# HeyWeCome/WhisprRec

Measured on AMD Instinct MI355X. Metric: BPR training triplets/sec, higher is better.
Workload: dtype f32; 1 GPU; BPRMF emb_size=64, synthetic 1000000 users x 1000000 items (uniform ids), batch 65536, SGD l2=0, plan build in timed region; batch=65536, emb_size=64, optimizer=SGD, plan_chunk_batches=64, tables=single GPU, step_stream=whisprrec_amd.hip_ops.PipelinedSgd, plan=group plan (no per-batch sort: flags + lists of the shared rows, wr_group.hip), chained_step_launch=True, plan_build=on a side stream, beside the steps of the chunk before

## Files before the change

include/whisprrec_hip.h:

```cpp
#ifndef WHISPRREC_HIP_H
#define WHISPRREC_HIP_H

#include <stdint.h>

#ifdef __cplusplus
extern "C" {
#endif

#define WR_ABI_VERSION 1

#define WR_OK 0
#define WR_E_NULL (-1)
#define WR_E_SHAPE (-2)
#define WR_E_WORKSPACE (-3)
#define WR_E_ALIGN (-4)
#define WR_E_RANGE (-5)

int32_t wr_abi_version(void);
const char *wr_last_error(void);
int32_t wr_device_info(int32_t *n_cu, int32_t *wave_size, char *arch, int32_t arch_len);

int64_t wr_bpr_fwd_workspace_bytes(int64_t B);
int32_t wr_bpr_fwd(const float *user_tab, int64_t n_users, const float *item_tab, int64_t n_items, int32_t D,
                   const int64_t *u, const int64_t *p, const int64_t *n, int64_t B, float *pos_score, float *neg_score,
// ... 143 lines not shown

int64_t wr_group_plan_words(int64_t n_triplets, int64_t batch_size, int64_t n_users, int64_t n_items);
int32_t wr_group_plan_layout(int64_t n_triplets, int64_t batch_size, int64_t n_users, int64_t n_items, int64_t *out);
int32_t wr_narrow_ids_i64(const int64_t *u, const int64_t *p, const int64_t *n, int32_t *u32, int32_t *p32, int32_t *n32,
                          int64_t count, void *stream);
int32_t wr_group_plan_build(const int32_t *u, const int32_t *p, const int32_t *n, int64_t n_triplets, int64_t batch_size,
                            int64_t n_users, int64_t n_items, int32_t *plan, int64_t plan_words, void *stream);
int64_t wr_bprmf_group_workspace_bytes(int64_t batch_size, int32_t D);
int64_t wr_bprmf_group_sync_words(int64_t n_batches);
int32_t wr_bprmf_group_supported(const float *user_tab, const float *item_tab, int32_t D);
int32_t wr_bprmf_run_sgd_group(float *user_tab, int64_t n_users, float *item_tab, int64_t n_items, int32_t D,
                               const int32_t *u, const int32_t *p, const int32_t *n, int64_t n_triplets, int64_t batch_size,
                               const int32_t *plan, int64_t plan_words, int64_t first_batch, int64_t n_batches, float lr,
                               float *loss_out, void *const *events, void *workspace, int64_t workspace_bytes, int32_t *sync,
                               int64_t sync_words, void *stream);

int32_t wr_bprmf_plan_overlap_marks(const int32_t *tu, const int32_t *tp, const int32_t *tn, int64_t n_triplets,
                                    int64_t batch_size, int64_t n_items, const int32_t *prev_bitmap, int32_t *bitmap,
                                    int32_t *tdef, int32_t *def_q, int64_t def_cap, int32_t *def_count, void *stream);

int32_t wr_bprmf_plan_overlap_deferred(const int32_t *tu, const int32_t *tp, const int32_t *tn, int64_t n_triplets,
                                       int64_t batch_size, int64_t n_items, const int32_t *prev_bitmap, const int32_t *bitmap,
                                       int32_t *tdef, int32_t *def_q, int64_t def_cap, int32_t *def_count, void *stream);

int32_t wr_bprmf_grads(const float *user_tab, int64_t n_users, const float *item_tab, int64_t n_items, int32_t D,
                       const int32_t *tu, const int32_t *tp, const int32_t *tn, const int32_t *oc_item,
                       const int32_t *oc_src, int64_t B, float *grad_u, float *grad_i, int32_t *stamp_u,
                       int32_t *stamp_i, int32_t step_id, float *loss_out, const wr_hot_runs *hot, void *workspace,
                       int64_t workspace_bytes, void *stream);

// ... 208 lines not shown
```

whisprrec_amd/abi.py:

```python
import ctypes
import os

_HERE = os.path.dirname(os.path.abspath(__file__))
LIB_PATH = os.path.join(_HERE, "libwhisprrec_hip.so")

c_i32, c_i64, c_f32, c_vp = ctypes.c_int32, ctypes.c_int64, ctypes.c_float, ctypes.c_void_p

SIGNATURES = {
    "wr_abi_version": (c_i32, []),
    "wr_last_error": (ctypes.c_char_p, []),
    "wr_device_info": (c_i32, [c_vp, c_vp, c_vp, c_i32]),
    "wr_bpr_fwd_workspace_bytes": (c_i64, [c_i64]),
    "wr_bpr_fwd": (c_i32, [c_vp, c_i64, c_vp, c_i64, c_i32, c_vp, c_vp, c_vp, c_i64, c_vp, c_vp, c_vp, c_vp, c_vp, c_i64,
                           c_vp]),
    "wr_bprmf_plan_workspace_bytes": (c_i64, [c_i64, c_i64, c_i64, c_i64]),
    "wr_bprmf_plan_build_i64": (c_i32, [c_vp, c_vp, c_vp, c_i64, c_i64, c_i64, c_i64, c_vp, c_vp, c_vp, c_vp, c_vp, c_vp,
                                        c_vp, c_vp, c_i64, c_vp]),
    "wr_bprmf_plan_build_i32": (c_i32, [c_vp, c_vp, c_vp, c_i64, c_i64, c_i64, c_i64, c_vp, c_vp, c_vp, c_vp, c_vp, c_vp,
                                        c_vp, c_vp, c_i64, c_vp]),
    "wr_bprmf_plan_small_max_batch": (c_i64, []),
    "wr_bprmf_plan_build_small_i64": (c_i32, [c_vp, c_vp, c_vp, c_i64, c_i64, c_i64, c_i64, c_vp, c_vp, c_vp, c_vp, c_vp, c_vp,
                                              c_vp, c_vp]),
    "wr_bprmf_plan_build_small_i32": (c_i32, [c_vp, c_vp, c_vp, c_i64, c_i64, c_i64, c_i64, c_vp, c_vp, c_vp, c_vp, c_vp, c_vp,
                                              c_vp, c_vp]),
# ... 48 lines not shown
                                 c_i64, c_f32, c_i32, c_vp, c_vp, c_vp, c_vp, c_i64, c_vp]),
    "wr_shard_route": (c_i32, [c_vp, c_vp, c_vp, c_i64, c_i64, c_i32, c_i32, c_i64, c_i64, c_i64, c_i64, c_i64, c_vp, c_vp, c_vp,
                               c_vp, c_vp, c_vp, c_vp]),
    "wr_shard_pack": (c_i32, [c_vp, c_vp, c_i64, c_i32, c_i64, c_i64, c_vp, c_i64, c_vp, c_vp, c_vp]),
    "wr_bprmf_shard_step_group": (c_i32, [c_vp, c_i64, c_vp, c_i64, c_i64, c_i32, c_vp, c_vp, c_vp, c_i64, c_i64, c_vp, c_i64,
                                          c_i64, c_i64, c_f32, c_vp, c_vp, c_vp, c_i64, c_vp, c_i64, c_vp]),
    "wr_group_plan_words": (c_i64, [c_i64, c_i64, c_i64, c_i64]),
    "wr_group_plan_layout": (c_i32, [c_i64, c_i64, c_i64, c_i64, c_vp]),
    "wr_narrow_ids_i64": (c_i32, [c_vp, c_vp, c_vp, c_vp, c_vp, c_vp, c_i64, c_vp]),
    "wr_group_plan_build": (c_i32, [c_vp, c_vp, c_vp, c_i64, c_i64, c_i64, c_i64, c_vp, c_i64, c_vp]),
    "wr_bprmf_group_workspace_bytes": (c_i64, [c_i64, c_i32]),
    "wr_bprmf_group_sync_words": (c_i64, [c_i64]),
    "wr_bprmf_group_supported": (c_i32, [c_vp, c_vp, c_i32]),
    "wr_bprmf_run_sgd_group": (c_i32, [c_vp, c_i64, c_vp, c_i64, c_i32, c_vp, c_vp, c_vp, c_i64, c_i64, c_vp, c_i64, c_i64,
                                       c_i64, c_f32, c_vp, c_vp, c_vp, c_i64, c_vp, c_i64, c_vp]),
    "wr_bprmf_plan_overlap_deferred": (c_i32, [c_vp, c_vp, c_vp, c_i64, c_i64, c_i64, c_vp, c_vp, c_vp, c_vp, c_i64, c_vp,
                                               c_vp]),
    "wr_bprmf_plan_fast_marks_supported": (c_i32, [c_i64, c_i64, c_i64, c_i64]),
    "wr_bprmf_plan_build_fast_marks_i64": (c_i32, [c_vp, c_vp, c_vp, c_i64, c_i64, c_i64, c_i64, c_vp, c_vp, c_vp, c_vp, c_vp,
                                                   c_vp, c_vp, c_vp, c_i64, c_vp, c_vp]),
    "wr_bprmf_plan_build_fast_marks_i32": (c_i32, [c_vp, c_vp, c_vp, c_i64, c_i64, c_i64, c_i64, c_vp, c_vp, c_vp, c_vp, c_vp,
                                                   c_vp, c_vp, c_vp, c_i64, c_vp, c_vp]),
    "wr_bprmf_plan_overlap_marks": (c_i32, [c_vp, c_vp, c_vp, c_i64, c_i64, c_i64, c_vp, c_vp, c_vp, c_vp, c_i64, c_vp,
                                            c_vp]),
    "wr_bprmf_grads": (c_i32, [c_vp, c_i64, c_vp, c_i64, c_i32, c_vp, c_vp, c_vp, c_vp, c_vp, c_i64, c_vp, c_vp, c_vp,
                               c_vp, c_i32, c_vp, c_vp, c_vp, c_i64, c_vp]),
    "wr_sgd_decay_untouched": (c_i32, [c_vp, c_i64, c_i32, c_vp, c_i32, c_f32, c_f32, c_vp]),
    "wr_sgd_dense": (c_i32, [c_vp, c_i64, c_i32, c_vp, c_vp, c_i32, c_f32, c_f32, c_vp]),
    "wr_adam_dense": (c_i32, [c_vp, c_vp, c_vp, c_i64, c_i32, c_vp, c_vp, c_i32, c_i64, c_f32, c_f32, c_f32, c_f32,
                              c_f32, c_vp]),
# ... 77 lines not shown



class HotRuns(ctypes.Structure):
    _fields_ = [("piece_q", c_vp), ("piece_len", c_vp), ("run_q", c_vp), ("run_first", c_vp), ("run_np", c_vp),
                ("u_piece_q", c_vp), ("u_piece_len", c_vp), ("u_run_q", c_vp), ("u_run_first", c_vp), ("u_run_np", c_vp),
                ("counts_host", c_vp), ("cap_pieces", c_i64), ("cap_runs", c_i64), ("cap_u_pieces", c_i64),
                ("cap_u_runs", c_i64)]


class DenseGroup(ctypes.Structure):
    _fields_ = [("A_T", c_vp), ("cols", c_vp), ("rows", c_vp), ("partials", c_vp), ("K_pad", c_i64), ("k_per_split", c_i64),
                ("n_tiles", c_i64)]


class BucketSide(ctypes.Structure):
    _fields_ = [("n_buckets", c_i32), ("row_bucket", c_vp), ("bucket_start", c_vp), ("bucket_rows", c_vp), ("bucket_sub", c_vp)]


_lib = None


class WhisprRecHipError(RuntimeError):
    pass


def lib():
    global _lib
    if _lib is None:
        if not os.path.exists(LIB_PATH):
# ... 29 lines not shown
```

whisprrec_amd/csrc/wr_group.hip:

```cpp
#include "wr_common.h"
#include <hip/hip_ext.h>

#include <algorithm>

namespace wr {

constexpr int kGpThreads = 1024;
constexpr unsigned kGpRangeBits = 18;
constexpr int kGpWords = 1 << (kGpRangeBits - 5);
constexpr int kGpCap = 8192;
constexpr int kGpBins = 4096;
constexpr int kGpMaxBin = 256;
constexpr int kGpMaxRanges = 8;
constexpr int64_t kGpMaxBatch = 1 << 17;
constexpr int kGpLongRun = 64;
constexpr int kGpMetaWords = 16;
#ifndef WR_GP_DBG
#define WR_GP_DBG 0
#endif

struct GroupLayout {
    int64_t nb, B, fw;
    int R_u, R_i, cap_u, cap_i;
    unsigned mask_u, mask_i, hbits_u, hbits_i;
// ... 669 lines not shown
#define WR_GS_NIT 1024
#endif

struct GroupRun {
    TablePair tabs;
    const int32_t *u, *p, *n, *plan;
    int64_t n_triplets, batch_size, plan_words, workspace_bytes, sync_words;
    BatchRange range;
    float lr, *loss_out;
    void *const *events;
    void *workspace;
    uint32_t *sync;
    int n_cu;
    float *grad_slots;
    int64_t n_local_items, global_batch;
    hipStream_t stream;
};

template <int T, int NV, bool FULL>
static int32_t launch_group_steps(const GroupRun &g, const GroupLayout &L, const GpDev &G) {
    const int32_t D = g.tabs.D;
    const int64_t n_batches = g.range.n_batches, global_batch = g.global_batch;
    uint32_t *const sync = g.sync;
    const int64_t B = L.B;
    const int64_t ws_one = gs_ws_one(B, D), zb = align_up(B * (int64_t)D * 4, 256);
    char *ws = reinterpret_cast<char *>(g.workspace);
    float *Zs[2] = {reinterpret_cast<float *>(ws), reinterpret_cast<float *>(ws + ws_one)};
    float *ZUs[2] = {reinterpret_cast<float *>(ws + zb), reinterpret_cast<float *>(ws + ws_one + zb)};
    float *Ps[2] = {reinterpret_cast<float *>(ws + 2 * zb), reinterpret_cast<float *>(ws + ws_one + 2 * zb)};
    constexpr int TEAMS = kBlock / T;
    WR_HIP(hipMemsetAsync(sync, 0, (size_t)(n_batches * kGsStepWords) * 4, g.stream));
    uint32_t *timeout = sync + (g.sync_words - 4);
    int nDS = WR_GS_NDS;
    while (nDS > g.n_cu / 4 && nDS > 1) nDS >>= 1;
    auto batch_of = [&](int64_t b) {
        const int64_t off = b * B;
        const int Bk = (int)batch_len(g.n_triplets, B, b);
        return GsBatch{g.u + off, g.p + off, g.n + off, reinterpret_cast<const uint4 *>(G.flags + b * L.fw * 4),
                       G.ul_row + b * L.R_u * (int64_t)L.cap_u, G.ul_src + b * L.R_u * (int64_t)L.cap_u, G.ucnt + b * L.R_u,
                       G.il_row + b * L.R_i * (int64_t)L.cap_i, G.il_src + b * L.R_i * (int64_t)L.cap_i, G.icnt + b * L.R_i,
                       Bk, L.R_u, L.R_i, L.cap_u, L.cap_i};
    };
    auto ev = [&](int64_t k, int j) { return g.events ? reinterpret_cast<hipEvent_t>(g.events[2 * k + j]) : (hipEvent_t) nullptr; };
    int n_partials_prev = 0;
    for (int64_t k = 0; k <= n_batches; ++k) {
        GsArgs a{};
        a.U = g.tabs.U;
        a.I = g.tabs.I;
        a.D = D;
        a.lr = g.lr;
        a.done = sync + (k < n_batches ? k : 0) * kGsStepWords;
        a.timeout = timeout;
        a.Gs = g.grad_slots;
        a.nL = (int)g.n_local_items;
        const bool have_cur = k < n_batches, have_prev = k > 0;
        if (have_cur) {
            a.cur = batch_of(g.range.first_batch + k);
            a.Z = Zs[k & 1];
            a.ZU = ZUs[k & 1];
            a.partials = Ps[k & 1];
            a.denom = global_batch > 0 ? (float)global_batch : (float)a.cur.B;
            a.nA = (int)((a.cur.B + TEAMS - 1) / TEAMS);
            a.nDS = have_prev ? nDS : 0;
            a.chained = have_prev ? 1 : 0;
        }
        if (have_prev) {
            a.prev = batch_of(g.range.first_batch + k - 1);
            a.Zp = Zs[(k - 1) & 1];
            a.ZUp = ZUs[(k - 1) & 1];
            a.partials_prev = Ps[(k - 1) & 1];
            a.n_partials_prev = n_partials_prev;
            a.denom_prev = global_batch > 0 ? (float)global_batch : (float)a.prev.B;
            a.loss_prev = at_or_null(g.loss_out, k - 1);
            a.nIT = (int)std::min<int64_t>(WR_GS_NIT, (2 * B + kGsTile - 1) / kGsTile + L.R_i);
            a.nUT = (int)std::min<int64_t>(WR_GS_NUT, (B + kGsTile - 1) / kGsTile + L.R_u);
        }
        a.tiles_at = (int)((int64_t)a.nA * WR_GS_TILES_AT / 16);
        a.side_at = std::max(a.tiles_at, (int)((int64_t)a.nA * WR_GS_SIDE_AT / 16));
        const dim3 grid((unsigned)(a.nA + a.nIT + a.nUT + a.nDS));
        hipEvent_t e0 = have_cur ? ev(k, 0) : nullptr, e1 = have_cur ? ev(k, 1) : nullptr;
        if (e0 != nullptr || e1 != nullptr)
            hipExtLaunchKernelGGL((bprmf_group_step<T, NV, FULL>), grid, dim3(kBlock), 0, g.stream, e0, e1, 0, a);
        else
            hipLaunchKernelGGL((bprmf_group_step<T, NV, FULL>), grid, dim3(kBlock), 0, g.stream, a);
        WR_LAUNCH_CHECK("bprmf_group_step");
        n_partials_prev = a.nA + a.nDS;
    }
    return WR_OK;
}

static int32_t check_group_plan(const char *entry, const GroupRun &g, GroupLayout &L) {
    int32_t rc;
    if ((rc = check_whole_lines(entry, whole_lines(g.tabs.U, g.tabs.I, g.tabs.D), g.tabs.D)) != WR_OK) return rc;
    WR_REQUIRE(group_layout(g.n_triplets, g.batch_size, g.tabs.n_users, g.tabs.n_items, L), WR_E_RANGE,
               "group plan not applicable to n=%lld, batch=%lld", (long long)g.n_triplets, (long long)g.batch_size);
    WR_REQUIRE(g.plan_words >= L.total, WR_E_WORKSPACE, "group plan: %lld words < %lld", (long long)g.plan_words, (long long)L.total);
    return WR_OK;
}

static int32_t run_group(const char *entry, GroupRun &g, const GroupLayout &L, int64_t sync_batches) {
    int32_t rc;
    if ((rc = check_workspace(entry, g.workspace, g.workspace_bytes, 2 * gs_ws_one(g.batch_size, g.tabs.D))) != WR_OK) return rc;
    if ((rc = check_sync_words(entry, g.sync, g.sync_words, sync_batches * kGsStepWords + 4)) != WR_OK) return rc;
    if (g.range.n_batches == 0) return WR_OK;
    if (g.n_cu == 0 && (rc = device_cu_count(&g.n_cu)) != WR_OK) return rc;
    const GpDev G = group_dev(const_cast<int32_t *>(g.plan), L);
#define WR_CALL_GS(T_, NV_, FULL_) return launch_group_steps<T_, NV_, FULL_>(g, L, G)
    WR_DISPATCH_D(g.tabs.D, WR_CALL_GS);
#undef WR_CALL_GS
    return WR_OK;
}

}

using namespace wr;

extern "C" {

int64_t wr_group_plan_words(int64_t n_triplets, int64_t batch_size, int64_t n_users, int64_t n_items) {
    GroupLayout L;
    if (!group_layout(n_triplets, batch_size, n_users, n_items, L)) return 0;
// ... 66 lines not shown
    g.plan = plan; g.plan_words = plan_words;
    g.range = BatchRange{first_batch, n_batches};
    g.lr = lr; g.loss_out = loss_out; g.events = events;
    g.workspace = workspace; g.workspace_bytes = workspace_bytes;
    g.sync = reinterpret_cast<uint32_t *>(sync); g.sync_words = sync_words;
    g.stream = reinterpret_cast<hipStream_t>(stream);
    int32_t rc;
    GroupLayout L;
    if ((rc = check_tables(g.tabs)) != WR_OK) return rc;
    WR_REQUIRE(u && p && n && plan && sync, WR_E_NULL, "index arrays / plan / sync words must not be NULL");
    if ((rc = check_group_plan("wr_bprmf_run_sgd_group", g, L)) != WR_OK) return rc;
    WR_REQUIRE(first_batch >= 0 && n_batches >= 0 && first_batch + n_batches <= L.nb, WR_E_SHAPE,
               "batches [%lld,%lld) exceed the plan's %lld", (long long)first_batch, (long long)(first_batch + n_batches),
               (long long)L.nb);
    return run_group("wr_bprmf_run_sgd_group", g, L, n_batches + 1);
}

int32_t wr_bprmf_shard_step_group(float *user_shard, int64_t n_user_rows, float *item_ext, int64_t n_ext_rows,
                                  int64_t n_local_items, int32_t D, const int32_t *vu, const int32_t *vp, const int32_t *vn,
                                  int64_t n_triplets, int64_t batch_size, const int32_t *plan, int64_t plan_words, int64_t batch,
                                  int64_t global_batch, float lr, float *grad_slots, float *loss_partial, void *workspace,
                                  int64_t workspace_bytes, int32_t *sync, int64_t sync_words, void *stream) {
    GroupRun g{};
    g.tabs = TablePair{user_shard, item_ext, n_user_rows, n_ext_rows, D};
    g.u = vu; g.p = vp; g.n = vn; g.n_triplets = n_triplets; g.batch_size = batch_size;
    g.plan = plan; g.plan_words = plan_words;
    g.range = BatchRange{batch, 1};
    g.lr = lr; g.loss_out = loss_partial;
    g.workspace = workspace; g.workspace_bytes = workspace_bytes;
    g.sync = reinterpret_cast<uint32_t *>(sync); g.sync_words = sync_words;
// ... 19 lines not shown
```

whisprrec_amd/hip_ops.py:

```python
import ctypes

import torch

from . import abi


def _stream():
    return torch.cuda.current_stream().cuda_stream


def _p(t):
    return None if t is None else t.data_ptr()


def _addr(struct):
    return ctypes.addressof(struct) if struct is not None else None


def _event_handles(events, per_step, count, allow_none):
    if events is None:
        return None
    if len(events) != per_step * count:
        raise ValueError("%s must hold %d events per step" % ("phase_events" if per_step == 4 else "events", per_step))
    handles = []
# ... 522 lines not shown

    def __init__(self, u, p, n, batch_size, n_users, n_items, arena=None, defer=False):
        u, p, n = (_req(t, torch.int32, nm, 1) for t, nm in ((u, "u"), (p, "p"), (n, "n")))
        N = u.numel()
        if not (p.numel() == N and n.numel() == N) or N == 0:
            raise ValueError("u/p/n must have the same non-zero length")
        L = abi.lib()
        self.u, self.p, self.n = u, p, n
        self.n_triplets, self.batch_size = N, int(batch_size)
        self.n_users, self.n_items = int(n_users), int(n_items)
        self.n_batches = (N + self.batch_size - 1) // self.batch_size
        self.words = int(L.wr_group_plan_words(N, self.batch_size, self.n_users, self.n_items))
        if self.words <= 0:
            raise abi.WhisprRecHipError("group plan: shape not supported (batch size %d)" % self.batch_size)
        self.arena = arena
        self._stream = torch.cuda.current_stream(u.device)
        if arena is not None:
            if arena.buf.numel() < self.words or arena.batch_size != self.batch_size or \
                    (arena.n_users, arena.n_items) != (self.n_users, self.n_items):
                raise ValueError("plan does not fit its arena")
            if arena.free is not None:
                self._stream.wait_event(arena.free)
                arena.free = None
            self.buf = arena.buf
            self._pinned = arena.meta_host
        else:
            self.buf = torch.empty(self.words, dtype=torch.int32, device=u.device)
            self._pinned = None
        abi.check(L.wr_group_plan_build(_p(u), _p(p), _p(n), N, self.batch_size, self.n_users, self.n_items, _p(self.buf),
                                        self.buf.numel(), _stream()), "wr_group_plan_build")
# ... 193 lines not shown
        return bufs[-1]

    def run_sgd_group(self, gplan, first, count, lr, losses=None, events=None):
        L = abi.lib()
        nbytes = abi.check_size(L.wr_bprmf_group_workspace_bytes(gplan.batch_size, self.D), "wr_bprmf_group_workspace_bytes")
        ws = workspace(self.dev, "group_step").get(nbytes)
        losses = self._loss_buf(losses, count)
        ev = _event_handles(events, 2, count, False)
        sync = self._group_sync(count)
        abi.check(L.wr_bprmf_run_sgd_group(*self._table_head(), _p(gplan.u), _p(gplan.p), _p(gplan.n), gplan.n_triplets,
                                           gplan.batch_size, _p(gplan.buf), gplan.buf.numel(), first, count, lr, _p(losses),
                                           _addr(ev), _p(ws), ws.numel(), _p(sync), sync.numel(), _stream()),
                  "wr_bprmf_run_sgd_group")
        self.step_id += count
        return losses

    def grads(self, plan, k, grad_u, grad_i, loss_out=None, stamps=True):
        L = abi.lib()
        ws = self._ws(plan.batch_size)
        su, si = self._stamps() if stamps else (None, None)
        loss_out = self._loss_buf(loss_out)
        self.step_id += 1
        hot = plan.hot_struct(k)
        abi.check(L.wr_bprmf_grads(*self._table_head(), *self._plan_ptrs(plan, k), _p(grad_u), _p(grad_i), _p(su), _p(si),
                                   self.step_id, _p(loss_out), _addr(hot), _p(ws), ws.numel(), _stream()), "wr_bprmf_grads")
        return loss_out, self.step_id


PAIR_SET_MIN_PAIRS = 1 << 20

# ... 293 lines not shown
    if adjacent:
        return torch.as_strided(a, (end - a.storage_offset(),), (1,), a.storage_offset())
    return torch.cat(ts)


class PipelinedSgd:

    PREFETCH_AFTER_TRIPLETS = 0
    PLAN_TRIPLETS = 1 << 22
    GROUP_MIN_ROWS_PER_TRIPLET = 12
    GROUP_MIN_BATCH = 4096

    CHAIN_MIN_BATCH = 8192
    CHAIN_MIN_ITEMS_PER_TRIPLET = 6

    def __init__(self, chunk=64, min_triplets=None, chain=True, inline_plan=False, group=True):
        import sys
        self.ops = sys.modules[__name__]
        self.chunk = int(chunk)
        self.chain = bool(chain)
        self.group = bool(group)
        self.inline_plan = inline_plan
        self.stats = {"plain_calls": 0, "chain_calls": 0, "group_calls": 0, "group_fallbacks": 0}
        self._garenas = {}
        if min_triplets is not None:
            self.PLAN_TRIPLETS = int(min_triplets)
        self.plan_stream = None
        self._arenas = {}

    def chunk_batches(self, batch_size):
        return max(self.chunk, self.PLAN_TRIPLETS // max(int(batch_size), 1))

    def _arena_pair(self, device, B, nb_total, overlap_items):
        cap = min(self.chunk_batches(B), max(int(nb_total), 1)) * B
        key = (str(device), B, int(overlap_items))
        pair = self._arenas.get(key)
        if pair is None or pair[0].max_triplets < cap:
            pair = [self.ops.PlanArena(device, cap, B, overlap_items=overlap_items) for _ in range(2)]
            self._arenas[key] = pair
        return pair

    def _garena_pair(self, device, B, nb_total, n_users, n_items):
        cap = min(self.chunk_batches(B), max(int(nb_total), 1)) * B
        key = (str(device), B, int(n_users), int(n_items))
        pair = self._garenas.get(key)
        if pair is None or pair[0].max_triplets < cap:
            pair = [self.ops.GroupArena(device, cap, B, n_users, n_items) for _ in range(2)]
            self._garenas[key] = pair
        return pair

    def plan(self, U, segments, batch, first_chunk=None, lr=None, prep=None, runner=None):
        if self.plan_stream is None:
            self.plan_stream = side_stream(U.device)
        B = int(batch)
        segs, first = [], 0
        for k, (rows, u, p, n) in enumerate(segments):
            nb = (u.numel() + B - 1) // B
            if u.numel() % B != 0 and any(s[1].numel() for s in segments[k + 1:]):
                raise ValueError("only the last segment may end with a short batch")
            segs.append({"tabs": self.ops.BprmfTables(U, rows) if nb else None, "nb": nb, "first": first})
            first += nb
        live = [s for s in segments if s[1].numel()]
# ... 3 lines not shown
        use_chain = self.chain and (runner is None or getattr(runner, "wants_chain_marks", False)) and \
            B >= self.CHAIN_MIN_BATCH and first >= 2 and \
            min([s[0].shape[0] for s in live] or [0]) >= self.CHAIN_MIN_ITEMS_PER_TRIPLET * B and \
            all(sg["tabs"].chain_supported() for sg in segs if sg["tabs"] is not None)
        min_rows = min([U.shape[0]] + [s[0].shape[0] for s in live])
        use_group = self.group and runner is None and len(live) == 1 and first >= 2 and \
            self.GROUP_MIN_BATCH <= B <= 131072 and u_all.dtype in (torch.int32, torch.int64) and \
            min_rows >= self.GROUP_MIN_ROWS_PER_TRIPLET * B and \
            all(sg["tabs"].group_supported() for sg in segs if sg["tabs"] is not None)
        garenas = self._garena_pair(U.device, B, first, U.shape[0], n_items) if use_group else None
        arenas = None if use_group else self._arena_pair(U.device, B, first, n_items if use_chain else 0)
        for a in (arenas or []) + (garenas or []):
            a.release_after(main)
        h = {"segs": segs, "B": B, "u": u_all, "p": p_all, "n": n_all, "nb": first, "n_users": U.shape[0], "n_items": n_items,
             "at": 0, "tag": 0, "next": None, "cur": None, "map": None, "arenas": arenas, "pos": 0,
             "group": use_group, "garenas": garenas, "device": U.device,
             "ids32": [torch.empty(u_all.numel(), dtype=torch.int32, device=U.device) for _ in range(3)]
                      if use_group and u_all.dtype == torch.int64 else None,
             "chain": use_chain, "prep": prep, "runner": runner, "inline": bool(self.inline_plan),
             "lead": [int(c) for c in (first_chunk if isinstance(first_chunk, (list, tuple)) else [first_chunk or 0]) if c]}
        self.plan_stream.wait_stream(main)
        self._prefetch(h)
        return h

    def _build_stream(self, h):
        return torch.cuda.current_stream(h["u"].device) if h["inline"] else self.plan_stream

    def _prefetch(self, h):
        if h["at"] >= h["nb"]:
            h["next"] = None
            return
# ... 1 lines not shown
        c = min(self.chunk_batches(B), h["nb"] - first)
        if h["lead"]:
            c = min(c, h["lead"].pop(0))
        h["at"] += c
        lo, hi = first * B, min(h["u"].numel(), (first + c) * B)
        with torch.cuda.stream(self._build_stream(h)):
            bmap = h["map"] if h["map"] else None
            if h["prep"] is not None:
                h["prep"].fill(lo, hi)
            if h["group"]:
                cols = (h["u"], h["p"], h["n"])
                if h["ids32"] is not None:
                    abi.check(abi.lib().wr_narrow_ids_i64(*[_p(c[lo:hi]) for c in cols], *[_p(c[lo:hi]) for c in h["ids32"]],
                                                          hi - lo, _stream()), "wr_narrow_ids_i64")
                    cols = h["ids32"]
                plan = self.ops.GroupPlan(cols[0][lo:hi], cols[1][lo:hi], cols[2][lo:hi], B, h["n_users"], h["n_items"],
                                          arena=h["garenas"][h["tag"]], defer=True)
                h["tag"] ^= 1
                h["next"] = (first, plan)
                return
            if h["arenas"] is None:
                h["arenas"] = self._arena_pair(h["device"], B, h["nb"], h["n_items"] if h["chain"] else 0)
            plan = self.ops.BatchPlan(h["u"][lo:hi], h["p"][lo:hi], h["n"][lo:hi], B, h["n_users"], h["n_items"],
                                      validate=False, ws_tag="rot%d" % h["tag"], bucket_map=bmap, arena=h["arenas"][h["tag"]],
                                      defer=True, overlap=h["chain"])
        h["tag"] ^= 1
        h["next"] = (first, plan)

    STICKY_MSG = "a wait inside a step launch expired (hand-off between the workgroups of one launch): the tables are not " \
                 "valid — do not save or evaluate them; restart the run"

    def _queue_sticky(self, h, tabs, main):
        words = tabs.sticky_words()
        if not words:
            return
        pin = h.get("sticky_pin")
        if pin is None or pin.numel() < 2 * len(words):
            pin = h["sticky_pin"] = torch.zeros(2 * max(len(words), 4), dtype=torch.int32, pin_memory=True)
        half = pin.numel() // 2
        off = half * (h.get("sticky_tag", 0) & 1)
        h["sticky_tag"] = h.get("sticky_tag", 0) + 1
        for j, wd in enumerate(words):
            pin[off + j:off + j + 1].copy_(wd, non_blocking=True)
        ev = torch.cuda.Event()
        ev.record(main)
        self._check_sticky(h)
        h["sticky_pending"] = (ev, pin[off:off + len(words)])

    def _check_sticky(self, h):
        pend = h.pop("sticky_pending", None)
        if pend is not None:
            pend[0].synchronize()
            if bool(pend[1].numpy().any()):
                raise abi.WhisprRecHipError(self.STICKY_MSG)

    def _take_next(self, h, pos, main):
        self._check_sticky(h)
        if h["next"] is None:
            self._prefetch(h)
        cur = h["next"]
        assert cur is not None and cur[0] == pos, "steps must be run in order"
        plan = cur[1]
        plan.validate()
        if isinstance(plan, GroupPlan):
            if plan.overflow or plan.long_run:
                h["group"] = False
                self.stats["group_fallbacks"] += 1
                if h["next"] is not None and h["next"][0] != cur[0]:
                    raise AssertionError("plan pipeline out of step")
                if plan.overflow:
                    first, B = cur[0], h["B"]
                    lo, hi = first * B, first * B + plan.n_triplets
                    plan.arena.release_after(main)
                    if h["arenas"] is None:
                        h["arenas"] = self._arena_pair(h["device"], B, h["nb"], h["n_items"] if h["chain"] else 0)
                    with torch.cuda.stream(self._build_stream(h)):
                        plan = self.ops.BatchPlan(h["u"][lo:hi], h["p"][lo:hi], h["n"][lo:hi], B, h["n_users"], h["n_items"],
                                                  validate=False, ws_tag="rot%d" % h["tag"], arena=h["arenas"][h["tag"]],
                                                  defer=True, overlap=h["chain"])
                    h["tag"] ^= 1
                    plan.validate()
                    cur = (first, plan)
            main.wait_event(plan.ready)
            h["cur"], h["next"] = cur, None
            return cur
        main.wait_event(plan.ready)
        if plan.fast_overflowed:
# ... 17 lines not shown
        while pos < end:
            cur = h["cur"]
            if cur is None or pos >= cur[0] + cur[1].n_batches:
                cur = self._take_next(h, pos, main)
            base, plan = cur
            c = min(end, base + plan.n_batches) - pos
            if h["inline"] and h["next"] is None and h["at"] < h["nb"]:
                mid = base + plan.n_batches // 2
                if pos >= mid:
                    self._prefetch(h)
                else:
                    c = min(c, mid - pos)
            elif self.PREFETCH_AFTER_TRIPLETS > 0 and h["next"] is None and h["at"] < h["nb"] and \
                    c > (self.PREFETCH_AFTER_TRIPLETS + h["B"] - 1) // h["B"]:
                c = (self.PREFETCH_AFTER_TRIPLETS + h["B"] - 1) // h["B"]
            if isinstance(plan, GroupPlan):
                sg["tabs"].run_sgd_group(plan, pos - base, c, lr, losses=losses[loss_off:loss_off + c])
                self.stats["group_calls"] += 1
            elif h["runner"] is not None:
                h["runner"](plan, pos - base, c, losses[loss_off:loss_off + c])
                self.stats["plain_calls"] += 1
            elif h["chain"] and plan.overlap is not None and c >= 2:
                sg["tabs"].run_sgd_chain(plan, pos - base, c, lr, losses=losses[loss_off:loss_off + c])
                self.stats["chain_calls"] += 1
            else:
                sg["tabs"].run_sgd(plan, pos - base, c, lr, losses=losses[loss_off:loss_off + c])
                self.stats["plain_calls"] += 1
            pos += c
            loss_off += c
            if pos >= base + plan.n_batches:
                plan.arena.release_after(main)
                self._queue_sticky(h, sg["tabs"], main)
            if h["next"] is None and not h["inline"]:
                self._prefetch(h)
        h["pos"] = pos

    def run(self, handle, seg, lr, losses):
        sg = handle["segs"][seg]
        if sg["nb"] == 0:
            return
        self._run_span(handle, sg, sg["first"], sg["first"] + sg["nb"], lr, losses, 0)
        if seg == len(handle["segs"]) - 1:
            self._check_sticky(handle)

    def run_steps(self, handle, count, lr, losses):
        assert len(handle["segs"]) == 1, "run_steps: single-segment handles"
        sg = handle["segs"][0]
        pos = handle["pos"]
        if pos + count > sg["nb"]:
            raise ValueError("run_steps: %d steps asked, %d left" % (count, sg["nb"] - pos))
        self._run_span(handle, sg, pos, pos + count, lr, losses, 0)


class LazyOptimizerState:

    FOLD_MAX_GAP = 40

    MAX_LAG = 64
    LAG_MIN_GAP = 64

    def __init__(self, tabs, name, lr, l2, betas=(0.9, 0.999), eps=1e-8, fold=None, max_lag=None):
        self.chain, self.chain_calls = True, 0
        if name not in ("SGD", "Adam"):
            raise ValueError(name)
        self.tabs, self.name, self.lr, self.l2, self.betas, self.eps = tabs, name, float(lr), float(l2), betas, float(eps)
        self.fold = fold if fold is None else bool(fold)
# ... 477 lines not shown
```

Baseline: 2.587 billion triplets/s.

## Carry the last batch's deferred update across group-plan chunk boundaries

The chained group step normally finishes the previous batch's scatter inside the next batch's kernel, but each call drained the pipeline with a tail launch at the chunk end. A carry struct now holds the last batch's plan pointers, buffer half and partial counts, so the next chunk's first step applies it chained instead of in a standalone drain. Each plan is built with one lead-in batch so row-sharing lists cover the boundary, and a third arena keeps the carried plan alive. A flush entry point drains the carry on fallback, lr or table change, and at run end. It also batches the sticky-word device-to-host copies into one copy, at the cost of more bookkeeping and a larger plan per chunk.

After: 2.633 billion triplets/s (median of 6 runs). 1.02x the previous value.

```diff
diff --git a/include/whisprrec_hip.h b/include/whisprrec_hip.h
--- a/include/whisprrec_hip.h
+++ b/include/whisprrec_hip.h
@@ -181,6 +181,31 @@
                                const int32_t *plan, int64_t plan_words, int64_t first_batch, int64_t n_batches, float lr,
                                float *loss_out, void *const *events, void *workspace, int64_t workspace_bytes, int32_t *sync,
                                int64_t sync_words, void *stream);
+
+typedef struct wr_group_carry {
+    const int32_t *u, *p, *n;
+    const void *flags;
+    const int32_t *ul_row, *ul_src, *ul_cnt, *il_row, *il_src, *il_cnt;
+    int32_t B, R_u, R_i, cap_u, cap_i;
+    int32_t valid;
+    int32_t half;
+    int32_t n_partials;
+    float denom, lr;
+    float *loss;
+    const void *user_tab, *item_tab, *workspace;
+    int32_t D;
+    int32_t reserved;
+    int64_t batch_size;
+} wr_group_carry;
+int32_t wr_bprmf_run_sgd_group_carry(float *user_tab, int64_t n_users, float *item_tab, int64_t n_items, int32_t D,
+                                     const int32_t *u, const int32_t *p, const int32_t *n, int64_t n_triplets,
+                                     int64_t batch_size, const int32_t *plan, int64_t plan_words, int64_t first_batch,
+                                     int64_t n_batches, float lr, float *loss_out, void *const *events, void *workspace,
+                                     int64_t workspace_bytes, int32_t *sync, int64_t sync_words, wr_group_carry *carry,
+                                     int32_t carry_in, int32_t carry_out, void *stream);
+int32_t wr_bprmf_group_flush(float *user_tab, int64_t n_users, float *item_tab, int64_t n_items, int32_t D, int64_t batch_size,
+                             void *workspace, int64_t workspace_bytes, int32_t *sync, int64_t sync_words,
+                             wr_group_carry *carry, void *stream);
 
 int32_t wr_bprmf_plan_overlap_marks(const int32_t *tu, const int32_t *tp, const int32_t *tn, int64_t n_triplets,
                                     int64_t batch_size, int64_t n_items, const int32_t *prev_bitmap, int32_t *bitmap,
diff --git a/whisprrec_amd/abi.py b/whisprrec_amd/abi.py
--- a/whisprrec_amd/abi.py
+++ b/whisprrec_amd/abi.py
@@ -86,6 +86,9 @@
     "wr_bprmf_group_supported": (c_i32, [c_vp, c_vp, c_i32]),
     "wr_bprmf_run_sgd_group": (c_i32, [c_vp, c_i64, c_vp, c_i64, c_i32, c_vp, c_vp, c_vp, c_i64, c_i64, c_vp, c_i64, c_i64,
                                        c_i64, c_f32, c_vp, c_vp, c_vp, c_i64, c_vp, c_i64, c_vp]),
+    "wr_bprmf_run_sgd_group_carry": (c_i32, [c_vp, c_i64, c_vp, c_i64, c_i32, c_vp, c_vp, c_vp, c_i64, c_i64, c_vp, c_i64, c_i64,
+                                             c_i64, c_f32, c_vp, c_vp, c_vp, c_i64, c_vp, c_i64, c_vp, c_i32, c_i32, c_vp]),
+    "wr_bprmf_group_flush": (c_i32, [c_vp, c_i64, c_vp, c_i64, c_i32, c_i64, c_vp, c_i64, c_vp, c_i64, c_vp, c_vp]),
     "wr_bprmf_plan_overlap_deferred": (c_i32, [c_vp, c_vp, c_vp, c_i64, c_i64, c_i64, c_vp, c_vp, c_vp, c_vp, c_i64, c_vp,
                                                c_vp]),
     "wr_bprmf_plan_fast_marks_supported": (c_i32, [c_i64, c_i64, c_i64, c_i64]),
@@ -193,6 +196,14 @@
                 ("n_tiles", c_i64)]
 
 
+class GroupCarry(ctypes.Structure):
+    _fields_ = [("u", c_vp), ("p", c_vp), ("n", c_vp), ("flags", c_vp), ("ul_row", c_vp), ("ul_src", c_vp), ("ul_cnt", c_vp),
+                ("il_row", c_vp), ("il_src", c_vp), ("il_cnt", c_vp), ("B", c_i32), ("R_u", c_i32), ("R_i", c_i32),
+                ("cap_u", c_i32), ("cap_i", c_i32), ("valid", c_i32), ("half", c_i32), ("n_partials", c_i32),
+                ("denom", c_f32), ("lr", c_f32), ("loss", c_vp), ("user_tab", c_vp), ("item_tab", c_vp), ("workspace", c_vp),
+                ("D", c_i32), ("reserved", c_i32), ("batch_size", c_i64)]
+
+
 class BucketSide(ctypes.Structure):
     _fields_ = [("n_buckets", c_i32), ("row_bucket", c_vp), ("bucket_start", c_vp), ("bucket_rows", c_vp), ("bucket_sub", c_vp)]
 
diff --git a/whisprrec_amd/csrc/wr_group.hip b/whisprrec_amd/csrc/wr_group.hip
--- a/whisprrec_amd/csrc/wr_group.hip
+++ b/whisprrec_amd/csrc/wr_group.hip
@@ -707,22 +707,29 @@
     int n_cu;
     float *grad_slots;
     int64_t n_local_items, global_batch;
+    wr_group_carry *carry;
+    bool carry_in, carry_out;
     hipStream_t stream;
 };
+
+static inline GsBatch batch_of_carry(const wr_group_carry &c) {
+    return GsBatch{c.u, c.p, c.n, reinterpret_cast<const uint4 *>(c.flags), c.ul_row, c.ul_src, c.ul_cnt, c.il_row, c.il_src,
+                   c.il_cnt, c.B, c.R_u, c.R_i, c.cap_u, c.cap_i};
+}
 
 template <int T, int NV, bool FULL>
 static int32_t launch_group_steps(const GroupRun &g, const GroupLayout &L, const GpDev &G) {
     const int32_t D = g.tabs.D;
     const int64_t n_batches = g.range.n_batches, global_batch = g.global_batch;
     uint32_t *const sync = g.sync;
-    const int64_t B = L.B;
+    const int64_t B = g.batch_size;
     const int64_t ws_one = gs_ws_one(B, D), zb = align_up(B * (int64_t)D * 4, 256);
     char *ws = reinterpret_cast<char *>(g.workspace);
     float *Zs[2] = {reinterpret_cast<float *>(ws), reinterpret_cast<float *>(ws + ws_one)};
     float *ZUs[2] = {reinterpret_cast<float *>(ws + zb), reinterpret_cast<float *>(ws + ws_one + zb)};
     float *Ps[2] = {reinterpret_cast<float *>(ws + 2 * zb), reinterpret_cast<float *>(ws + ws_one + 2 * zb)};
     constexpr int TEAMS = kBlock / T;
-    WR_HIP(hipMemsetAsync(sync, 0, (size_t)(n_batches * kGsStepWords) * 4, g.stream));
+    if (n_batches > 0) WR_HIP(hipMemsetAsync(sync, 0, (size_t)(n_batches * kGsStepWords) * 4, g.stream));
     uint32_t *timeout = sync + (g.sync_words - 4);
     int nDS = WR_GS_NDS;
     while (nDS > g.n_cu / 4 && nDS > 1) nDS >>= 1;
@@ -735,8 +742,11 @@
                        Bk, L.R_u, L.R_i, L.cap_u, L.cap_i};
     };
     auto ev = [&](int64_t k, int j) { return g.events ? reinterpret_cast<hipEvent_t>(g.events[2 * k + j]) : (hipEvent_t) nullptr; };
-    int n_partials_prev = 0;
-    for (int64_t k = 0; k <= n_batches; ++k) {
+    const bool carried = g.carry != nullptr && g.carry_in;
+    const int h0 = carried ? (g.carry->half ^ 1) : 0;
+    int n_partials_prev = carried ? g.carry->n_partials : 0;
+    const int64_t k_end = (g.carry != nullptr && g.carry_out) ? n_batches - 1 : n_batches;
+    for (int64_t k = 0; k <= k_end; ++k) {
         GsArgs a{};
         a.U = g.tabs.U;
         a.I = g.tabs.I;
@@ -746,27 +756,28 @@
         a.timeout = timeout;
         a.Gs = g.grad_slots;
         a.nL = (int)g.n_local_items;
-        const bool have_cur = k < n_batches, have_prev = k > 0;
+        const bool have_cur = k < n_batches, have_prev = k > 0 || carried;
+        const int hk = (h0 + (int)(k & 1)) & 1;
         if (have_cur) {
             a.cur = batch_of(g.range.first_batch + k);
-            a.Z = Zs[k & 1];
-            a.ZU = ZUs[k & 1];
-            a.partials = Ps[k & 1];
+            a.Z = Zs[hk];
+            a.ZU = ZUs[hk];
+            a.partials = Ps[hk];
             a.denom = global_batch > 0 ? (float)global_batch : (float)a.cur.B;
             a.nA = (int)((a.cur.B + TEAMS - 1) / TEAMS);
             a.nDS = have_prev ? nDS : 0;
             a.chained = have_prev ? 1 : 0;
         }
         if (have_prev) {
-            a.prev = batch_of(g.range.first_batch + k - 1);
-            a.Zp = Zs[(k - 1) & 1];
-            a.ZUp = ZUs[(k - 1) & 1];
-            a.partials_prev = Ps[(k - 1) & 1];
+            a.prev = k > 0 ? batch_of(g.range.first_batch + k - 1) : batch_of_carry(*g.carry);
+            a.Zp = Zs[hk ^ 1];
+            a.ZUp = ZUs[hk ^ 1];
+            a.partials_prev = Ps[hk ^ 1];
             a.n_partials_prev = n_partials_prev;
-            a.denom_prev = global_batch > 0 ? (float)global_batch : (float)a.prev.B;
-            a.loss_prev = at_or_null(g.loss_out, k - 1);
-            a.nIT = (int)std::min<int64_t>(WR_GS_NIT, (2 * B + kGsTile - 1) / kGsTile + L.R_i);
-            a.nUT = (int)std::min<int64_t>(WR_GS_NUT, (B + kGsTile - 1) / kGsTile + L.R_u);
+            a.denom_prev = k > 0 ? (global_batch > 0 ? (float)global_batch : (float)a.prev.B) : g.carry->denom;
+            a.loss_prev = k > 0 ? at_or_null(g.loss_out, k - 1) : g.carry->loss;
+            a.nIT = (int)std::min<int64_t>(WR_GS_NIT, (2 * B + kGsTile - 1) / kGsTile + a.prev.R_i);
+            a.nUT = (int)std::min<int64_t>(WR_GS_NUT, (B + kGsTile - 1) / kGsTile + a.prev.R_u);
         }
         a.tiles_at = (int)((int64_t)a.nA * WR_GS_TILES_AT / 16);
         a.side_at = std::max(a.tiles_at, (int)((int64_t)a.nA * WR_GS_SIDE_AT / 16));
@@ -779,6 +790,28 @@
         WR_LAUNCH_CHECK("bprmf_group_step");
         n_partials_prev = a.nA + a.nDS;
     }
+    if (g.carry != nullptr) {
+        wr_group_carry &c = *g.carry;
+        if (g.carry_out) {
+            const GsBatch last = batch_of(g.range.first_batch + n_batches - 1);
+            c = wr_group_carry{};
+            c.u = last.u; c.p = last.p; c.n = last.n; c.flags = last.flags;
+            c.ul_row = last.ul_row; c.ul_src = last.ul_src; c.ul_cnt = last.ul_cnt;
+            c.il_row = last.il_row; c.il_src = last.il_src; c.il_cnt = last.il_cnt;
+            c.B = last.B; c.R_u = last.R_u; c.R_i = last.R_i; c.cap_u = last.cap_u; c.cap_i = last.cap_i;
+            c.valid = 1;
+            c.half = (h0 + (int)((n_batches - 1) & 1)) & 1;
+            c.n_partials = n_partials_prev;
+            c.denom = global_batch > 0 ? (float)global_batch : (float)last.B;
+            c.lr = g.lr;
+            c.loss = at_or_null(g.loss_out, n_batches - 1);
+            c.user_tab = g.tabs.U; c.item_tab = g.tabs.I; c.workspace = g.workspace;
+            c.D = D;
+            c.batch_size = B;
+        } else {
+            c = wr_group_carry{};
+        }
+    }
     return WR_OK;
 }
 
@@ -791,13 +824,35 @@
     return WR_OK;
 }
 
+static int32_t check_carry(const char *entry, const GroupRun &g) {
+    if (g.carry == nullptr) return WR_OK;
+    const wr_group_carry &c = *g.carry;
+    if (!g.carry_in) {
+        WR_REQUIRE(c.valid == 0, WR_E_RANGE, "%s: the carry holds a batch: flush it first (wr_bprmf_group_flush)", entry);
+        return WR_OK;
+    }
+    WR_REQUIRE(c.valid != 0, WR_E_RANGE, "%s: carry_in with an empty carry", entry);
+    WR_REQUIRE(c.user_tab == g.tabs.U && c.item_tab == g.tabs.I && c.D == g.tabs.D && c.workspace == g.workspace &&
+                   c.batch_size == g.batch_size,
+               WR_E_RANGE, "%s: the carry belongs to other tables, another workspace or another batch size", entry);
+    WR_REQUIRE(g.range.n_batches == 0 || c.lr == g.lr, WR_E_RANGE, "%s: lr %g differs from the carried batch's %g: flush first", entry,
+               (double)g.lr, (double)c.lr);
+    WR_REQUIRE(c.flags && c.ul_row && c.ul_src && c.ul_cnt && c.il_row && c.il_src && c.il_cnt && c.B > 0 && c.B <= g.batch_size &&
+                   c.R_u > 0 && c.R_u <= kGpMaxRanges && c.R_i > 0 && c.R_i <= kGpMaxRanges && (c.half == 0 || c.half == 1) &&
+                   c.n_partials >= 0 && c.n_partials <= (g.batch_size + teams_per_block(g.tabs.D) - 1) / teams_per_block(g.tabs.D) + 512,
+               WR_E_RANGE, "%s: the carry is damaged", entry);
+    return WR_OK;
+}
+
 static int32_t run_group(const char *entry, GroupRun &g, const GroupLayout &L, int64_t sync_batches) {
     int32_t rc;
     if ((rc = check_workspace(entry, g.workspace, g.workspace_bytes, 2 * gs_ws_one(g.batch_size, g.tabs.D))) != WR_OK) return rc;
     if ((rc = check_sync_words(entry, g.sync, g.sync_words, sync_batches * kGsStepWords + 4)) != WR_OK) return rc;
-    if (g.range.n_batches == 0) return WR_OK;
+    if ((rc = check_carry(entry, g)) != WR_OK) return rc;
+    if (g.range.n_batches == 0 && !(g.carry_in && !g.carry_out)) return WR_OK;
+    if (g.range.n_batches == 0) g.lr = g.carry->lr;
     if (g.n_cu == 0 && (rc = device_cu_count(&g.n_cu)) != WR_OK) return rc;
-    const GpDev G = group_dev(const_cast<int32_t *>(g.plan), L);
+    const GpDev G = g.plan != nullptr ? group_dev(const_cast<int32_t *>(g.plan), L) : GpDev{};
 #define WR_CALL_GS(T_, NV_, FULL_) return launch_group_steps<T_, NV_, FULL_>(g, L, G)
     WR_DISPATCH_D(g.tabs.D, WR_CALL_GS);
 #undef WR_CALL_GS
@@ -894,6 +949,54 @@
                "batches [%lld,%lld) exceed the plan's %lld", (long long)first_batch, (long long)(first_batch + n_batches),
                (long long)L.nb);
     return run_group("wr_bprmf_run_sgd_group", g, L, n_batches + 1);
+}
+
+int32_t wr_bprmf_run_sgd_group_carry(float *user_tab, int64_t n_users, float *item_tab, int64_t n_items, int32_t D,
+                                     const int32_t *u, const int32_t *p, const int32_t *n, int64_t n_triplets,
+                                     int64_t batch_size, const int32_t *plan, int64_t plan_words, int64_t first_batch,
+                                     int64_t n_batches, float lr, float *loss_out, void *const *events, void *workspace,
+                                     int64_t workspace_bytes, int32_t *sync, int64_t sync_words, wr_group_carry *carry,
+                                     int32_t carry_in, int32_t carry_out, void *stream) {
+    GroupRun g{};
+    g.tabs = TablePair{user_tab, item_tab, n_users, n_items, D};
+    g.u = u; g.p = p; g.n = n; g.n_triplets = n_triplets; g.batch_size = batch_size;
+    g.plan = plan; g.plan_words = plan_words;
+    g.range = BatchRange{first_batch, n_batches};
+    g.lr = lr; g.loss_out = loss_out; g.events = events;
+    g.workspace = workspace; g.workspace_bytes = workspace_bytes;
+    g.sync = reinterpret_cast<uint32_t *>(sync); g.sync_words = sync_words;
+    g.carry = carry; g.carry_in = carry_in != 0; g.carry_out = carry_out != 0;
+    g.stream = reinterpret_cast<hipStream_t>(stream);
+    int32_t rc;
+    GroupLayout L;
+    if ((rc = check_tables(g.tabs)) != WR_OK) return rc;
+    WR_REQUIRE(u && p && n && plan && sync, WR_E_NULL, "index arrays / plan / sync words must not be NULL");
+    WR_REQUIRE(carry != nullptr, WR_E_NULL, "carry is NULL");
+    if ((rc = check_group_plan("wr_bprmf_run_sgd_group_carry", g, L)) != WR_OK) return rc;
+    WR_REQUIRE(first_batch >= 0 && n_batches >= 0 && first_batch + n_batches <= L.nb, WR_E_SHAPE,
+               "batches [%lld,%lld) exceed the plan's %lld", (long long)first_batch, (long long)(first_batch + n_batches),
+               (long long)L.nb);
+    return run_group("wr_bprmf_run_sgd_group_carry", g, L, n_batches + 1);
+}
+
+int32_t wr_bprmf_group_flush(float *user_tab, int64_t n_users, float *item_tab, int64_t n_items, int32_t D, int64_t batch_size,
+                             void *workspace, int64_t workspace_bytes, int32_t *sync, int64_t sync_words,
+                             wr_group_carry *carry, void *stream) {
+    GroupRun g{};
+    g.tabs = TablePair{user_tab, item_tab, n_users, n_items, D};
+    g.batch_size = batch_size;
+    g.workspace = workspace; g.workspace_bytes = workspace_bytes;
+    g.sync = reinterpret_cast<uint32_t *>(sync); g.sync_words = sync_words;
+    g.carry = carry; g.carry_in = true; g.carry_out = false;
+    g.stream = reinterpret_cast<hipStream_t>(stream);
+    int32_t rc;
+    if ((rc = check_tables(g.tabs)) != WR_OK) return rc;
+    WR_REQUIRE(sync != nullptr, WR_E_NULL, "sync words must not be NULL");
+    WR_REQUIRE(carry != nullptr, WR_E_NULL, "carry is NULL");
+    if ((rc = check_whole_lines("wr_bprmf_group_flush", whole_lines(g.tabs.U, g.tabs.I, g.tabs.D), g.tabs.D)) != WR_OK) return rc;
+    WR_REQUIRE(batch_size > 0 && batch_size <= kGpMaxBatch, WR_E_RANGE, "group plan not applicable to batch=%lld", (long long)batch_size);
+    if (carry->valid == 0) return WR_OK;
+    return run_group("wr_bprmf_group_flush", g, GroupLayout{}, 1);
 }
 
 int32_t wr_bprmf_shard_step_group(float *user_shard, int64_t n_user_rows, float *item_ext, int64_t n_ext_rows,
diff --git a/whisprrec_amd/hip_ops.py b/whisprrec_amd/hip_ops.py
--- a/whisprrec_amd/hip_ops.py
+++ b/whisprrec_amd/hip_ops.py
@@ -560,6 +560,7 @@
         if self.words <= 0:
             raise abi.WhisprRecHipError("group plan: shape not supported (batch size %d)" % self.batch_size)
         self.arena = arena
+        self.lead_in = 0
         self._stream = torch.cuda.current_stream(u.device)
         if arena is not None:
             if arena.buf.numel() < self.words or arena.batch_size != self.batch_size or \
@@ -783,6 +784,29 @@
                   "wr_bprmf_run_sgd_group")
         self.step_id += count
         return losses
+
+    def run_sgd_group_carry(self, gplan, first, count, lr, carry, carry_in, carry_out, losses=None, events=None):
+        L = abi.lib()
+        nbytes = abi.check_size(L.wr_bprmf_group_workspace_bytes(gplan.batch_size, self.D), "wr_bprmf_group_workspace_bytes")
+        ws = workspace(self.dev, "group_step").get(nbytes)
+        losses = self._loss_buf(losses, count)
+        ev = _event_handles(events, 2, count, False)
+        sync = self._group_sync(count)
+        abi.check(L.wr_bprmf_run_sgd_group_carry(*self._table_head(), _p(gplan.u), _p(gplan.p), _p(gplan.n), gplan.n_triplets,
+                                                 gplan.batch_size, _p(gplan.buf), gplan.buf.numel(), first, count, lr,
+                                                 _p(losses), _addr(ev), _p(ws), ws.numel(), _p(sync), sync.numel(),
+                                                 ctypes.addressof(carry), int(bool(carry_in)), int(bool(carry_out)), _stream()),
+                  "wr_bprmf_run_sgd_group_carry")
+        self.step_id += count
+        return losses
+
+    def group_flush(self, carry, batch_size):
+        L = abi.lib()
+        nbytes = abi.check_size(L.wr_bprmf_group_workspace_bytes(batch_size, self.D), "wr_bprmf_group_workspace_bytes")
+        ws = workspace(self.dev, "group_step").get(nbytes)
+        sync = self._group_sync(0)
+        abi.check(L.wr_bprmf_group_flush(*self._table_head(), batch_size, _p(ws), ws.numel(), _p(sync), sync.numel(),
+                                         ctypes.addressof(carry), _stream()), "wr_bprmf_group_flush")
 
     def grads(self, plan, k, grad_u, grad_i, loss_out=None, stamps=True):
         L = abi.lib()
@@ -1106,14 +1130,15 @@
     CHAIN_MIN_BATCH = 8192
     CHAIN_MIN_ITEMS_PER_TRIPLET = 6
 
-    def __init__(self, chunk=64, min_triplets=None, chain=True, inline_plan=False, group=True):
+    def __init__(self, chunk=64, min_triplets=None, chain=True, inline_plan=False, group=True, carry=True):
         import sys
         self.ops = sys.modules[__name__]
+        self.carry = bool(carry)
         self.chunk = int(chunk)
         self.chain = bool(chain)
         self.group = bool(group)
         self.inline_plan = inline_plan
-        self.stats = {"plain_calls": 0, "chain_calls": 0, "group_calls": 0, "group_fallbacks": 0}
+        self.stats = {"plain_calls": 0, "chain_calls": 0, "group_calls": 0, "group_fallbacks": 0, "group_flushes": 0}
         self._garenas = {}
         if min_triplets is not None:
             self.PLAN_TRIPLETS = int(min_triplets)
@@ -1133,11 +1158,12 @@
         return pair
 
     def _garena_pair(self, device, B, nb_total, n_users, n_items):
-        cap = min(self.chunk_batches(B), max(int(nb_total), 1)) * B
+        cap = (min(self.chunk_batches(B), max(int(nb_total), 1)) + (1 if self.carry else 0)) * B
+        count = 3 if self.carry else 2
         key = (str(device), B, int(n_users), int(n_items))
         pair = self._garenas.get(key)
-        if pair is None or pair[0].max_triplets < cap:
-            pair = [self.ops.GroupArena(device, cap, B, n_users, n_items) for _ in range(2)]
+        if pair is None or pair[0].max_triplets < cap or len(pair) != count:
+            pair = [self.ops.GroupArena(device, cap, B, n_users, n_items) for _ in range(count)]
             self._garenas[key] = pair
         return pair
 
@@ -1171,7 +1197,8 @@
             a.release_after(main)
         h = {"segs": segs, "B": B, "u": u_all, "p": p_all, "n": n_all, "nb": first, "n_users": U.shape[0], "n_items": n_items,
              "at": 0, "tag": 0, "next": None, "cur": None, "map": None, "arenas": arenas, "pos": 0,
-             "group": use_group, "garenas": garenas, "device": U.device,
+             "group": use_group, "garenas": garenas, "gtag": 0, "device": U.device,
+             "carry": abi.GroupCarry() if use_group and self.carry else None, "carry_tabs": None, "carry_arena": None,
              "ids32": [torch.empty(u_all.numel(), dtype=torch.int32, device=U.device) for _ in range(3)]
                       if use_group and u_all.dtype == torch.int64 else None,
              "chain": use_chain, "prep": prep, "runner": runner, "inline": bool(self.inline_plan),
@@ -1203,10 +1230,13 @@
                     abi.check(abi.lib().wr_narrow_ids_i64(*[_p(c[lo:hi]) for c in cols], *[_p(c[lo:hi]) for c in h["ids32"]],
                                                           hi - lo, _stream()), "wr_narrow_ids_i64")
                     cols = h["ids32"]
-                plan = self.ops.GroupPlan(cols[0][lo:hi], cols[1][lo:hi], cols[2][lo:hi], B, h["n_users"], h["n_items"],
-                                          arena=h["garenas"][h["tag"]], defer=True)
-                h["tag"] ^= 1
-                h["next"] = (first, plan)
+                lead = 1 if h["carry"] is not None and first > 0 else 0
+                lo_p = lo - lead * B
+                plan = self.ops.GroupPlan(cols[0][lo_p:hi], cols[1][lo_p:hi], cols[2][lo_p:hi], B, h["n_users"], h["n_items"],
+                                          arena=h["garenas"][h["gtag"]], defer=True)
+                plan.lead_in = lead
+                h["gtag"] = (h["gtag"] + 1) % len(h["garenas"])
+                h["next"] = (first - lead, plan)
                 return
             if h["arenas"] is None:
                 h["arenas"] = self._arena_pair(h["device"], B, h["nb"], h["n_items"] if h["chain"] else 0)
@@ -1229,8 +1259,14 @@
         half = pin.numel() // 2
         off = half * (h.get("sticky_tag", 0) & 1)
         h["sticky_tag"] = h.get("sticky_tag", 0) + 1
-        for j, wd in enumerate(words):
-            pin[off + j:off + j + 1].copy_(wd, non_blocking=True)
+        if len(words) == 1:
+            pin[off:off + 1].copy_(words[0], non_blocking=True)
+        else:
+            dev_words = h.get("sticky_dev")
+            if dev_words is None or dev_words.numel() != len(words):
+                dev_words = h["sticky_dev"] = torch.empty(len(words), dtype=torch.int32, device=words[0].device)
+            torch.cat(words, out=dev_words)
+            pin[off:off + len(words)].copy_(dev_words, non_blocking=True)
         ev = torch.cuda.Event()
         ev.record(main)
         self._check_sticky(h)
@@ -1244,22 +1280,28 @@
                 raise abi.WhisprRecHipError(self.STICKY_MSG)
 
     def _take_next(self, h, pos, main):
-        self._check_sticky(h)
+        if h["carry"] is None:
+            self._check_sticky(h)
         if h["next"] is None:
             self._prefetch(h)
         cur = h["next"]
-        assert cur is not None and cur[0] == pos, "steps must be run in order"
+        assert cur is not None and cur[0] + getattr(cur[1], "lead_in", 0) == pos, "steps must be run in order"
         plan = cur[1]
-        plan.validate()
+        try:
+            plan.validate()
+        except IndexError:
+            self._flush(h)
+            raise
         if isinstance(plan, GroupPlan):
             if plan.overflow or plan.long_run:
+                self._flush(h)
                 h["group"] = False
                 self.stats["group_fallbacks"] += 1
                 if h["next"] is not None and h["next"][0] != cur[0]:
                     raise AssertionError("plan pipeline out of step")
                 if plan.overflow:
-                    first, B = cur[0], h["B"]
-                    lo, hi = first * B, first * B + plan.n_triplets
+                    first, B = cur[0] + plan.lead_in, h["B"]
+                    lo, hi = first * B, first * B + plan.n_triplets - plan.lead_in * B
                     plan.arena.release_after(main)
                     if h["arenas"] is None:
                         h["arenas"] = self._arena_pair(h["device"], B, h["nb"], h["n_items"] if h["chain"] else 0)
@@ -1307,7 +1349,19 @@
             elif self.PREFETCH_AFTER_TRIPLETS > 0 and h["next"] is None and h["at"] < h["nb"] and \
                     c > (self.PREFETCH_AFTER_TRIPLETS + h["B"] - 1) // h["B"]:
                 c = (self.PREFETCH_AFTER_TRIPLETS + h["B"] - 1) // h["B"]
-            if isinstance(plan, GroupPlan):
+            if not isinstance(plan, GroupPlan):
+                self._flush(h)
+            if isinstance(plan, GroupPlan) and h["carry"] is not None:
+                tabs, carry = sg["tabs"], h["carry"]
+                if carry.valid and (h["carry_tabs"] is not tabs or carry.lr != ctypes.c_float(lr).value or pos - base < 1):
+                    self._flush(h)
+                cin = bool(carry.valid)
+                tabs.run_sgd_group_carry(plan, pos - base, c, lr, carry, cin, True, losses=losses[loss_off:loss_off + c])
+                if cin and h["carry_arena"] is not plan.arena:
+                    h["carry_arena"].release_after(main)
+                h["carry_tabs"], h["carry_arena"] = tabs, plan.arena
+                self.stats["group_calls"] += 1
+            elif isinstance(plan, GroupPlan):
                 sg["tabs"].run_sgd_group(plan, pos - base, c, lr, losses=losses[loss_off:loss_off + c])
                 self.stats["group_calls"] += 1
             elif h["runner"] is not None:
@@ -1321,18 +1375,34 @@
                 self.stats["plain_calls"] += 1
             pos += c
             loss_off += c
+            h["pos"] = pos
             if pos >= base + plan.n_batches:
-                plan.arena.release_after(main)
+                if plan.arena is not h["carry_arena"]:
+                    plan.arena.release_after(main)
                 self._queue_sticky(h, sg["tabs"], main)
             if h["next"] is None and not h["inline"]:
                 self._prefetch(h)
         h["pos"] = pos
+
+    def _flush(self, h):
+        carry = h.get("carry")
+        if carry is None or not carry.valid:
+            return
+        h["carry_tabs"].group_flush(carry, h["B"])
+        self.stats["group_flushes"] += 1
+        arena, h["carry_arena"] = h["carry_arena"], None
+        cur = h["cur"]
+        if cur is not None and cur[1].arena is arena and h["pos"] < cur[0] + cur[1].n_batches:
+            return
+        if arena is not None:
+            arena.release_after(torch.cuda.current_stream(h["device"]))
 
     def run(self, handle, seg, lr, losses):
         sg = handle["segs"][seg]
         if sg["nb"] == 0:
             return
         self._run_span(handle, sg, sg["first"], sg["first"] + sg["nb"], lr, losses, 0)
+        self._flush(handle)
         if seg == len(handle["segs"]) - 1:
             self._check_sticky(handle)
 
@@ -1343,6 +1413,7 @@
         if pos + count > sg["nb"]:
             raise ValueError("run_steps: %d steps asked, %d left" % (count, sg["nb"] - pos))
         self._run_span(handle, sg, pos, pos + count, lr, losses, 0)
+        self._flush(handle)
 
 
 class LazyOptimizerState:
```
